# data-mermaid/mermaid-classifier

Measured on AMD Instinct MI355X. Metric: patches/sec (224x224 EfficientNet-B0), higher is better.
Workload: dtype f16; 1 GPU; EfficientNet-B0 forward, batch=256 random 224x224 u8 patches per GPU -> (256,1280) fp32; per_gpu_batch=256, global_batch=256, weights=synthetic seed 0, input_batches_rotated=8, lanes_per_gpu=2, parallelism=patch-sharded x1

## Files before the change

### include/mmc.h

```cpp
#ifndef MMC_H
#define MMC_H

#include <stddef.h>
#include <stdint.h>

#ifdef __cplusplus
extern "C" {
#endif

#define MMC_OK 0
#define MMC_ERR_ARG 1
#define MMC_ERR_WEIGHTS 2
#define MMC_ERR_HIP 3
#define MMC_ERR_NOMEM 4

#define MMC_ARCH_B0 0
#define MMC_ARCH_B4 1

#define MMC_IN_DEVICE 0u
#define MMC_IN_HOST 1u
#define MMC_OUT_DEVICE 0u
#define MMC_OUT_HOST 2u

#define MMC_FEATURE_DIM_B0 1280
#define MMC_FEATURE_DIM_B4 1792
#define MMC_PATCH 224

typedef struct mmc_backbone mmc_backbone;
typedef struct mmc_head mmc_head;

const char* mmc_last_error(void);
int mmc_version(void);
int mmc_device_count(void);

int mmc_backbone_create(const void* packed, size_t nbytes, int arch, int device, int max_batch,
                        mmc_backbone** out);
#define MMC_PRECISION_FP8 1u
int mmc_backbone_create_ex(const void* packed, size_t nbytes, int arch, int device, int max_batch, unsigned flags,
                           mmc_backbone** out);
int mmc_fp8_e4m3_encode(const float* in, uint8_t* out, size_t n);
void mmc_backbone_destroy(mmc_backbone* bb);
int mmc_feature_dim(const mmc_backbone* bb);
int mmc_backbone_max_batch(const mmc_backbone* bb);
int mmc_backbone_lanes(const mmc_backbone* bb);
size_t mmc_backbone_workspace_bytes(const mmc_backbone* bb);

int mmc_backbone_extract(mmc_backbone* bb, const void* patches, int64_t n, float* out_features,
                         unsigned flags, void* hip_stream);

int mmc_backbone_graph_stats(mmc_backbone* bb, int64_t stats[3]);

int mmc_backbone_read_activation(mmc_backbone* bb, const char* name, float* out, size_t capacity,
                                 size_t* n_written);

int mmc_backbone_profile(mmc_backbone* bb, const void* patches_dev, int64_t n, float* out_features_dev,
                         void* hip_stream, char (*names)[64], float* ms, int* launches, int cap, int* n_out);

int mmc_crop_patches(const void* image, int height, int width, const int32_t* rowcols, int64_t n,
                     void* patches_out_dev, unsigned flags, int device, void* hip_stream);

int mmc_head_create(const float* const* W, const float* const* b, const int* dims, int n_layers,
                    const float* a, const float* bcal, int K, int device, mmc_head** out);
void mmc_head_destroy(mmc_head* h);
int mmc_head_input_dim(const mmc_head* h);
int mmc_head_num_classes(const mmc_head* h);
int mmc_head_predict(mmc_head* h, const float* feats, int64_t n, float* proba, int32_t* argmax,
                     unsigned flags, void* hip_stream);

int mmc_head_topk(mmc_head* h, const float* feats, int64_t n, int k,
                  int32_t* idx , float* scores , float* proba ,
                  unsigned flags, void* hip_stream);

int mmc_classify_patches(mmc_backbone* bb, mmc_head* h, const void* patches, int64_t n, int k,
// ... 132 lines not shown
```

### mermaid_classifier_amd/_lib.py

```python

from __future__ import annotations

import ctypes as C
import os
from pathlib import Path

_HERE = Path(__file__).resolve().parent
LIB_NAME = "libmermaid_mi355.so"
LIB_PATH = _HERE / LIB_NAME

MMC_OK, MMC_ERR_ARG, MMC_ERR_WEIGHTS, MMC_ERR_HIP, MMC_ERR_NOMEM = 0, 1, 2, 3, 4
MMC_PRECISION_FP8 = 1
MMC_IN_HOST, MMC_OUT_HOST = 1, 2
MMC_EVAL_TOTALS = 5
MMC_GROUPED_MAX_BINS, MMC_COVER_SUMS = 64, 8
MMC_GROUPED_MAX_SOURCE_CELLS, MMC_GROUPED_MAX_COVER_CELLS = 1 << 26, 1 << 28
MMC_CATEGORY_MAX, MMC_CATEGORY_MAX_BINS = 64, 20
MMC_CATEGORY_MIN_BINS, MMC_CATEGORY_ROWS_PER_BIN = 2, 10
MMC_RANKED_MAX_K = 16
MMC_TRAINER_GROUP_MAX = 16

SYMBOLS = [
    "mmc_last_error", "mmc_version", "mmc_device_count",
    "mmc_backbone_create", "mmc_backbone_create_ex", "mmc_fp8_e4m3_encode", "mmc_backbone_destroy", "mmc_feature_dim", "mmc_backbone_max_batch", "mmc_backbone_lanes",
    "mmc_backbone_workspace_bytes", "mmc_backbone_extract", "mmc_backbone_read_activation",
    "mmc_backbone_profile", "mmc_backbone_graph_stats", "mmc_crop_patches",
    "mmc_head_create", "mmc_head_destroy", "mmc_head_input_dim", "mmc_head_num_classes", "mmc_head_predict", "mmc_head_topk", "mmc_classify_patches",
    "mmc_trainer_create", "mmc_trainer_destroy", "mmc_trainer_partial_fit", "mmc_trainer_partial_fit_ordered", "mmc_trainer_get_params", "mmc_trainer_adam_state",
    "mmc_trainer_logits", "mmc_trainer_evaluate", "mmc_trainer_evaluate_q32", "mmc_trainer_set_loss", "mmc_trainer_loss_gradient",
    "mmc_calibrator_create", "mmc_calibrator_destroy", "mmc_calibrator_add_features", "mmc_calibrator_add_scores", "mmc_calibrator_fit",
    "mmc_featureset_create", "mmc_featureset_destroy", "mmc_featureset_rows", "mmc_featureset_dim", "mmc_featureset_append", "mmc_featureset_read",
    "mmc_trainer_partial_fit_set", "mmc_trainer_group_partial_fit_set", "mmc_trainer_evaluate_set_q32", "mmc_calibrator_add_set",
    "mmc_trainer_evaluate_classes", "mmc_trainer_evaluate_classes_set",
    "mmc_head_evaluate", "mmc_head_evaluate_set", "mmc_head_evaluate_grouped", "mmc_head_evaluate_grouped_set",
    "mmc_head_evaluate_categories", "mmc_head_evaluate_categories_set",
    "mmc_head_evaluate_ranked", "mmc_head_evaluate_ranked_set",
    "mmc_dist_unique_id", "mmc_dist_create", "mmc_dist_destroy", "mmc_gather_features",
]


class LibraryMissingError(ImportError):
    pass


def _load() -> C.CDLL:
    path = Path(os.environ.get("MMC_LIBRARY", LIB_PATH))
    if not path.is_file():
        raise LibraryMissingError(
            f"{path} not found: build it with `python -m mermaid_classifier_amd.build` "
            "(hipcc --offload-arch=gfx950). mermaid_classifier_amd has no CPU fallback.")
    try:
        import torch
    except ImportError:
        pass
    lib = C.CDLL(str(path))
    vp, i32, i64, u32, sz = C.c_void_p, C.c_int, C.c_int64, C.c_uint, C.c_size_t
    fp = C.POINTER(C.c_float)
    lib.mmc_last_error.restype = C.c_char_p
    lib.mmc_last_error.argtypes = []
    lib.mmc_version.restype = i32
    lib.mmc_device_count.restype = i32
    lib.mmc_backbone_create.restype = i32
    lib.mmc_backbone_create.argtypes = [vp, sz, i32, i32, i32, C.POINTER(vp)]
    lib.mmc_backbone_create_ex.restype = i32
    lib.mmc_backbone_create_ex.argtypes = [vp, sz, i32, i32, i32, u32, C.POINTER(vp)]
    lib.mmc_fp8_e4m3_encode.restype = i32
    lib.mmc_fp8_e4m3_encode.argtypes = [vp, vp, sz]
    lib.mmc_backbone_destroy.restype = None
    lib.mmc_backbone_destroy.argtypes = [vp]
    lib.mmc_feature_dim.restype = i32
    lib.mmc_feature_dim.argtypes = [vp]
    lib.mmc_backbone_max_batch.restype = i32
    lib.mmc_backbone_max_batch.argtypes = [vp]
    lib.mmc_backbone_lanes.restype = i32
    lib.mmc_backbone_lanes.argtypes = [vp]
    lib.mmc_backbone_workspace_bytes.restype = sz
    lib.mmc_backbone_workspace_bytes.argtypes = [vp]
    lib.mmc_backbone_extract.restype = i32
    lib.mmc_backbone_extract.argtypes = [vp, vp, i64, vp, u32, vp]
    lib.mmc_backbone_read_activation.restype = i32
    lib.mmc_backbone_read_activation.argtypes = [vp, C.c_char_p, vp, sz, C.POINTER(sz)]
    lib.mmc_backbone_profile.restype = i32
    lib.mmc_backbone_profile.argtypes = [vp, vp, i64, vp, vp, vp, fp, C.POINTER(i32), i32, C.POINTER(i32)]
    lib.mmc_backbone_graph_stats.restype = i32
    lib.mmc_backbone_graph_stats.argtypes = [vp, C.POINTER(i64)]
    lib.mmc_crop_patches.restype = i32
    lib.mmc_crop_patches.argtypes = [vp, i32, i32, vp, i64, vp, u32, i32, vp]
    lib.mmc_head_create.restype = i32
    lib.mmc_head_create.argtypes = [C.POINTER(fp), C.POINTER(fp), C.POINTER(i32), i32, fp, fp, i32, i32, C.POINTER(vp)]
    lib.mmc_head_destroy.restype = None
    lib.mmc_head_destroy.argtypes = [vp]
    lib.mmc_head_input_dim.restype = i32
    lib.mmc_head_input_dim.argtypes = [vp]
    lib.mmc_head_num_classes.restype = i32
    lib.mmc_head_num_classes.argtypes = [vp]
    lib.mmc_head_predict.restype = i32
    lib.mmc_head_predict.argtypes = [vp, vp, i64, vp, vp, u32, vp]
    lib.mmc_head_topk.restype = i32
    lib.mmc_head_topk.argtypes = [vp, vp, i64, i32, vp, vp, vp, u32, vp]
    lib.mmc_classify_patches.restype = i32
# ... 110 lines not shown
```

### mermaid_classifier_amd/csrc/device_common.h

```cpp
#pragma once
#include <hip/hip_runtime.h>
#include <stdint.h>
#include <stdlib.h>
#include <algorithm>
#include <atomic>
#include <type_traits>

#include "kernels.h"

typedef _Float16 h8 __attribute__((ext_vector_type(8)));
typedef _Float16 h4 __attribute__((ext_vector_type(4)));
typedef float f4 __attribute__((ext_vector_type(4)));
typedef float f2 __attribute__((ext_vector_type(2)));

static __device__ __forceinline__ float sigmoid_f(float x) { return __builtin_amdgcn_rcpf(1.0f + __expf(-x)); }
static __device__ __forceinline__ float silu_f(float x) { return x * sigmoid_f(x); }
static __device__ __forceinline__ float silu_scaled(float t)
{
    return t * __builtin_amdgcn_rcpf(1.0f + __builtin_amdgcn_exp2f(-t));
}

static __device__ __forceinline__ uint32_t cvt_pk_f16(float a, float b)
{
    uint32_t d;
// ... 69 lines not shown
}

static __device__ __forceinline__ float fma_mix_lo(uint32_t h2, float w, float acc)
{
    float d;
    asm("v_fma_mix_f32 %0, %1, %2, %3 op_sel_hi:[1,0,0]" : "=v"(d) : "v"(h2), "v"(w), "v"(acc));
    return d;
}
static __device__ __forceinline__ float fma_mix_hi(uint32_t h2, float w, float acc)
{
    float d;
    asm("v_fma_mix_f32 %0, %1, %2, %3 op_sel:[1,0,0] op_sel_hi:[1,0,0]" : "=v"(d) : "v"(h2), "v"(w), "v"(acc));
    return d;
}


#define GLOBAL_AS __attribute__((address_space(1)))
typedef uint32_t u2v __attribute__((ext_vector_type(2)));
typedef uint32_t u4v __attribute__((ext_vector_type(4)));
template <typename T>
static __device__ __forceinline__ const GLOBAL_AS T* sgpr_ptr(const void* p)
{
    const uint64_t v = reinterpret_cast<uint64_t>(p);
    const uint32_t lo = __builtin_amdgcn_readfirstlane((uint32_t)v), hi = __builtin_amdgcn_readfirstlane((uint32_t)(v >> 32));
    return reinterpret_cast<const GLOBAL_AS T*>(((uint64_t)hi << 32) | lo);
}
template <typename T>
static __device__ __forceinline__ T gload(const GLOBAL_AS void* base, unsigned byte_off)
{
    return *reinterpret_cast<const GLOBAL_AS T*>(reinterpret_cast<const GLOBAL_AS char*>(base) + byte_off);
}
#define T7_BAR() asm volatile("s_waitcnt lgkmcnt(0)\n\ts_barrier" ::: "memory")

#define LAUNCH_CHECK()                          \
    do {                                        \
        hipError_t e__ = hipGetLastError();     \
        if (e__ != hipSuccess) return (int)e__; \
    } while (0)

template <auto Kernel>
static int set_max_lds(int bytes)
{
    static std::atomic<bool> done[64];
    int dev = 0;
    if (hipGetDevice(&dev) != hipSuccess) dev = 0;
    const bool tracked = dev >= 0 && dev < 64;
    if (tracked && done[dev].load(std::memory_order_acquire)) return 0;
    const hipError_t e = hipFuncSetAttribute(reinterpret_cast<const void*>(Kernel), hipFuncAttributeMaxDynamicSharedMemorySize, bytes);
    if (e != hipSuccess) return (int)e;
    if (tracked) done[dev].store(true, std::memory_order_release);
    return 0;
}

template <int NK, typename Args>
struct Inst {
    int key[NK];
    const char* label;
    int (*launch)(const Args&, hipStream_t);
};
template <int NK, typename Args, size_t N>
static const Inst<NK, Args>* find_inst(const Inst<NK, Args> (&table)[N], const int (&key)[NK])
{
    for (const auto& t : table)
        if (std::equal(key, key + NK, t.key)) return &t;
    return nullptr;
}
// ... 14 lines not shown
```

### mermaid_classifier_amd/csrc/k_early.hip

```cpp
#include "device_common.h"

template <int KSTEPS, bool RES>
__global__ __launch_bounds__(256) void thin_proj_kernel(const _Float16* __restrict__ X, int K, const _Float16* __restrict__ Wp,
                                                        const float* __restrict__ bias, _Float16* __restrict__ Y, int N,
                                                        const float* __restrict__ gate, int HW, int frags_per_wg,
                                                        const _Float16* __restrict__ res, int plane_rows)
{
    const int tid = threadIdx.x, lane = tid & 63, wave = tid >> 6;
    const int m = lane & 15, q = lane >> 4;
    const int b = blockIdx.y;
    const int nfrag = HW >> 4;
    const int f0 = blockIdx.x * frags_per_wg;
    const int f1 = f0 + frags_per_wg < nfrag ? f0 + frags_per_wg : nfrag;
    const int cbase = q * 8;
    const int cres = cbase < N ? cbase : 0;
    const _Float16* xb = X + (size_t)b * HW * K;
    auto load = [&](int f, h8 (&dst)[KSTEPS], h8& r) {
        const size_t row = (size_t)f * 16 + m;
#pragma unroll
        for (int ks = 0; ks < KSTEPS; ++ks) {
            const int k0 = ks * 32 + q * 8, k = k0 < K ? k0 : K - 8;
            dst[ks] = plane_rows ? *reinterpret_cast<const h8*>(X + (((size_t)(k >> 5) * plane_rows + (size_t)b * HW + row) * 32 + (k & 31)))
                                 : *reinterpret_cast<const h8*>(xb + row * K + k);
        }
// ... 30 lines not shown
        if (more) load(f + 4, xn, rn);
        f4 a0 = bv0, a1 = bv1;
#pragma unroll
        for (int ks = 0; ks < KSTEPS; ++ks) {
            a0 = __builtin_amdgcn_mfma_f32_16x16x32_f16(wf[ks][0], xc[ks], a0, 0, 0, 0);
            a1 = __builtin_amdgcn_mfma_f32_16x16x32_f16(wf[ks][1], xc[ks], a1, 0, 0, 0);
        }
        if (cbase < N) {
            h8 o;
#pragma unroll
            for (int j = 0; j < 4; ++j) {
                o[j] = (_Float16)(a0[j] + (RES ? (float)rc[j] : 0.f));
                o[4 + j] = (_Float16)(a1[j] + (RES ? (float)rc[4 + j] : 0.f));
            }
            *reinterpret_cast<h8*>(Y + ((size_t)b * HW + (size_t)f * 16 + m) * N + cbase) = o;
        }
        if (more) {
#pragma unroll
            for (int ks = 0; ks < KSTEPS; ++ks) xc[ks] = xn[ks];
            rc = rn;
        }
    }
}

template <bool PLANAR>
__global__ __launch_bounds__(512, 4) void mb1_kernel(Mb1Args a)
{
    constexpr int WC = 58, NPOS = 17 * WC, NPF = (NPOS + 15) / 16, ES2 = 160;
    extern __shared__ __attribute__((aligned(16))) unsigned char smem[];
    unsigned char* E = smem;
    float* pred = reinterpret_cast<float*>(smem + NPF * 8 * ES2);
    const int tid = threadIdx.x, lane = tid & 63, wave = __builtin_amdgcn_readfirstlane(tid >> 6);
    const int m = lane & 15, q = lane >> 4;
    const int tile = blockIdx.x, b = blockIdx.z;
    const int ty = tile >> 1, tx = tile & 1;
    const int oy0 = 8 * ty, ox0 = 28 * tx, iy0 = 16 * ty, ix0 = 56 * tx;
    const GLOBAL_AS _Float16* xg = sgpr_ptr<_Float16>(a.X) + (size_t)b * 112 * 112 * 32;
    uint2 xbp[8];
    {
        u4v xr[8];
#pragma unroll
        for (int i = 0; i < 8; ++i) {
            const int pf = wave + 8 * i;
            const int p = 16 * pf + m;
            const int r = p / WC, c = p - r * WC;
            const int iy = iy0 + r, ix = ix0 + c;
            const bool ok = pf < NPF && p < NPOS && iy < 112 && ix < 112;
            xr[i] = gload<u4v>(xg, (unsigned)((((ok ? iy : 0) * 112 + (ok ? ix : 0)) * 32 + 8 * q) * 2));
        }
        const uint4 wraw = *reinterpret_cast<const uint4*>(a.pre_w + lane * 8);
        const f4 bpre = *reinterpret_cast<const f4*>(a.pre_b + 4 * q);
        const f4 g0 = *reinterpret_cast<const f4*>(a.pre_gate + (size_t)b * 32 + 8 * q);
        const f4 g1 = *reinterpret_cast<const f4*>(a.pre_gate + (size_t)b * 32 + 8 * q + 4);
        const uint4 wgated = gate_h8(wraw, g0, g1);
        const h8 wpre = *reinterpret_cast<const h8*>(&wgated);
#pragma unroll
        for (int i = 0; i < 8; ++i) {
            const f4 x1 = __builtin_amdgcn_mfma_f32_16x16x32_f16(wpre, *reinterpret_cast<const h8*>(&xr[i]), bpre, 0, 0, 0);
            h4 xh;
#pragma unroll
            for (int j = 0; j < 4; ++j) xh[j] = (_Float16)x1[j];
            xbp[i] = *reinterpret_cast<const uint2*>(&xh);
        }
    }
    h4 wexp[2];
    float bexp[2];
    float kdw[9], dbias;
// ... 85 lines not shown
            for (int j = 0; j < 14; j += 2) {
                const f2 v = {acc[j], acc[j + 1]};
                psum2 = psum2 + v;
                const uint32_t hv = cvt_pk_f16(acc[j], acc[j + 1]);
                dg[(size_t)j * PS] = (uint16_t)hv;
                dg[(size_t)(j + 1) * PS] = (uint16_t)(hv >> 16);
            }
            pred[(tid >> 5) * 32 + c] = psum2.x + psum2.y;
        }
        T7_BAR();
        if (tid < 32) {
            float s = 0.f;
#pragma unroll
            for (int w = 0; w < 16; ++w) s += pred[w * 32 + tid];
            a.pool[((size_t)b * 14 + tile) * 96 + chunk * 32 + tid] = s;
        }
    }
}

template <int KSD, int CKS, int CE, int HIMG>
__global__ __launch_bounds__(512) void mbt_kernel(MbtArgs a)
{
    constexpr int R = KSD / 2, NP = KSD == 5 ? 3 : 2, NROWS = 14 + 2 * R, CH = 48;
    constexpr int ES2 = 224;
    constexpr int WW = HIMG == 28 ? 28 : 30;
    constexpr int NPOS = NROWS * WW, NPF = (NPOS + 15) / 16;
    static_assert(NPF <= 32, "four fragments per wave");
    constexpr int TX = HIMG / 28, NR = 3 + 2 * R;
    extern __shared__ __attribute__((aligned(16))) unsigned char smem[];
    unsigned char* E = smem;
    float* pred = reinterpret_cast<float*>(smem + NPF * 8 * ES2);
    const int tid = threadIdx.x, lane = tid & 63, wave = __builtin_amdgcn_readfirstlane(tid >> 6);
    const int m = lane & 15, q = lane >> 4;
    const int tile = blockIdx.x, chunk = blockIdx.y, b = blockIdx.z;
    const int ty = tile / TX, tx = tile - ty * TX;
    const int oy0 = 14 * ty, ox0 = 28 * tx;
    const int wx0 = ox0 >= 2 ? ox0 - 2 : 0;
    const int Cin = a.Cin;
    const GLOBAL_AS _Float16* xg = sgpr_ptr<_Float16>(a.X) + (size_t)b * HIMG * HIMG * Cin;
    const GLOBAL_AS _Float16* wexp = sgpr_ptr<_Float16>(a.wexp);
    uint32_t raw[15];
    float dbias;
    const int cg_dw = chunk * CH + tid % CH;
    {
        u4v xr[4][CKS];
        constexpr bool MASK_E = KSD != 3;
        bool okp[4][2];
#pragma unroll
        for (int i = 0; i < 4; ++i) {
            const int p = 16 * (wave + 8 * i) + m;
            const int r = p / WW, c = p - r * WW;
            const int iy = oy0 - R + r, ix = wx0 + c;
            const bool ok = p < NPOS && iy >= 0 && iy < HIMG && ix < HIMG;
            const int row = ok ? iy * HIMG + ix : 0;
#pragma unroll
            for (int h = 0; h < 2; ++h) {
                const int pp = 16 * (wave + 8 * i) + 4 * q + 2 * h;
                const int pr = pp / WW, pc = pp - pr * WW;
                const int py = oy0 - R + pr;
                okp[i][h] = !MASK_E || (pp < NPOS && py >= 0 && py < HIMG && wx0 + pc < HIMG);
            }
#pragma unroll
            for (int ks = 0; ks < CKS; ++ks) {
                const int kk = 32 * ks + 8 * q;
                xr[i][ks] = gload<u4v>(xg, (unsigned)((row * Cin + (kk < Cin ? kk : Cin - 8)) * 2));
            }
        }
// ... 86 lines not shown
                            const bool out = ro == 0 ? (oy0 + rb == 0) : (oy0 + rb + 1 == HIMG - 1);
                            wq[0][0] = out ? 0u : wq[0][0]; wq[0][1] = out ? 0u : wq[0][1];
                            wq[1][0] = out ? 0u : wq[1][0]; wq[1][1] = out ? 0u : wq[1][1];
                        }
                    }
#pragma unroll
                    for (int ip = 0; ip < NP; ++ip)
#pragma unroll
                        for (int j = 0; j < 14; ++j) {
                            const int l = (KSD == 5 || !(j & 1)) ? (j >> 1) + ip : (j >> 1) + 1 + ip;
                            if (ky == 0 && ip == 0) acc[j] = dot2_from(P[ro + ky][l], wq[j & 1][ip], dbias);
                            else acc[j] = __builtin_amdgcn_fdot2(*reinterpret_cast<const h2*>(&P[ro + ky][l]),
                                                                 *reinterpret_cast<const h2*>(&wq[j & 1][ip]), acc[j], false);
                        }
                }
                silu_scaled_staged(acc);
#pragma unroll
                for (int j = 0; j < 14; j += 2) {
                    const f2 v = {acc[j], acc[j + 1]};
                    psum2 = psum2 + v;
                    const uint32_t hv = cvt_pk_f16(acc[j], acc[j + 1]);
                    reinterpret_cast<uint16_t*>(dg)[((size_t)ro * HIMG + j) * CE] = (uint16_t)hv;
                    reinterpret_cast<uint16_t*>(dg)[((size_t)ro * HIMG + j + 1) * CE] = (uint16_t)(hv >> 16);
                }
            }
        }
        pred[rest * CH + c] = psum2.x + psum2.y;
    }
    T7_BAR();
    if (tid < CH) {
        float s = 0.f;
#pragma unroll
        for (int w = 0; w < 10; ++w) s += pred[w * CH + tid];
        a.pool[((size_t)b * gridDim.x + tile) * CE + chunk * CH + tid] = s;
    }
}

template <int CKS, int CE>
__global__ __launch_bounds__(512, 4) void mbt4_kernel(MbtArgs a)
{
    constexpr int HIMG = 28, R = 2, KSD = 5, NROWS = 18, WW = 28, CH = 48, NPOS = NROWS * WW, NPF = 32;
    constexpr int ERS = 64, ECS = 1160;
    constexpr int TREG = 56 * 32;
    extern __shared__ __attribute__((aligned(16))) unsigned char smem[];
    unsigned char* E = smem;
    const int tid = threadIdx.x, lane = tid & 63, wave = __builtin_amdgcn_readfirstlane(tid >> 6);
    unsigned char* TW = smem + CH * ECS + wave * TREG;
    float* pred = reinterpret_cast<float*>(smem + CH * ECS + 8 * TREG);
    const int m = lane & 15, q = lane >> 4;
    const int tile = blockIdx.x, chunk = blockIdx.y, b = blockIdx.z;
    const int oy0 = 14 * tile;
    const int Cin = a.Cin;
    const GLOBAL_AS _Float16* xg = sgpr_ptr<_Float16>(a.X) + (size_t)b * HIMG * HIMG * Cin;
    const GLOBAL_AS _Float16* wexp = sgpr_ptr<_Float16>(a.wexp);
    const GLOBAL_AS _Float16* dwt = sgpr_ptr<_Float16>(a.dwtoe);
    {
        u4v xr[4][CKS];
        int eoff[4];
        bool okq[4];
#pragma unroll
        for (int i = 0; i < 4; ++i) {
            const int p = 16 * (wave + 8 * i) + m;
            const int r = (p * 2341) >> 16, c = p - r * WW;
            const int iy = oy0 - R + r;
            const bool ok = p < NPOS && iy >= 0 && iy < HIMG;
            const int row = ok ? iy * HIMG + c : 0;
            const int pq = 16 * (wave + 8 * i) + 4 * q;
            const int qr = (pq * 2341) >> 16, qc = pq - qr * WW;
            const int qy = oy0 - R + qr;
            okq[i] = pq < NPOS && qy >= 0 && qy < HIMG;
            eoff[i] = pq < NPOS ? qr * ERS + qc * 2 : NROWS * ERS;
#pragma unroll
            for (int ks = 0; ks < CKS; ++ks) {
                const int kk = 32 * ks + 8 * q;
                xr[i][ks] = gload<u4v>(xg, (unsigned)((row * Cin + (kk < Cin ? kk : Cin - 8)) * 2));
            }
        }
        h8 wa[3][CKS];
        float ba[3];
#pragma unroll
        for (int nf = 0; nf < 3; ++nf) {
            const int nfg = 3 * chunk + nf;
#pragma unroll
// ... 98 lines not shown
            }
            float v[14];
#pragma unroll
            for (int x = 0; x < 14; ++x) v[x] = XH == 0 ? acc[(x + 2) >> 2][(x + 2) & 3] : acc[x >> 2][x & 3];
            silu_scaled_staged(v);
            float s = ((v[0] + v[1]) + (v[2] + v[3])) + ((v[4] + v[5]) + (v[6] + v[7])) + ((v[8] + v[9]) + (v[10] + v[11])) + (v[12] + v[13]);
            s = quad_sum(rowok ? s : 0.f);
            if (n == 0) pred[(2 * yt + xh) * CH + 16 * g + c] = s;
#pragma unroll
            for (int j = 0; j < 7; ++j) {
                float lo = v[j], hi = v[7 + j];
                asm volatile("s_nop 1\n\tv_permlane16_swap_b32 %0, %1\n\ts_nop 1" : "+v"(lo), "+v"(hi));
                *reinterpret_cast<uint32_t*>(tst + j * 32) = cvt_pk_f16(lo, hi);
            }
#pragma unroll
            for (int rr = 0; rr < 2; ++rr) {
                const uint4 o = *reinterpret_cast<const uint4*>(TW + toff[rr]);
                *reinterpret_cast<uint4*>(dgb + goff[rr] + 32 * g) = o;
            }
        };
        if (xh == 0) {
#pragma unroll
            for (int g = 0; g < 3; ++g) item(g, std::integral_constant<int, 0>{});
        } else {
#pragma unroll
            for (int g = 0; g < 3; ++g) item(g, std::integral_constant<int, 1>{});
        }
    }
    T7_BAR();
    if (tid < CH) {
        float s = 0.f;
#pragma unroll
        for (int w = 0; w < 8; ++w) s += pred[w * CH + tid];
        a.pool[((size_t)b * gridDim.x + tile) * CE + chunk * CH + tid] = s;
    }
}

template <int KSD, int CKS, int CE, int HIMG>
__global__ __launch_bounds__(512) void mbt2_kernel(MbtArgs a)
{
    constexpr int PADB = KSD == 5 ? 1 : 0, NIP = KSD == 5 ? 3 : 2, NROWS = 12 + KSD, CH = 48, ES2 = 224;
    constexpr int WW = KSD == 5 ? 32 : 30, NPOS = NROWS * WW, NPF = (NPOS + 15) / 16, NS = (NPF + 7) / 8;
    constexpr int HOUT = HIMG / 2, TX = HOUT / 14, NPR = KSD == 5 ? 16 : 15;
    extern __shared__ __attribute__((aligned(16))) unsigned char smem[];
    unsigned char* E = smem;
    float* pred = reinterpret_cast<float*>(smem + NS * 64 * ES2);
    const int tid = threadIdx.x, lane = tid & 63, wave = __builtin_amdgcn_readfirstlane(tid >> 6);
    const int m = lane & 15, q = lane >> 4;
    const int tile = blockIdx.x, chunk = blockIdx.y, b = blockIdx.z;
    const int ty = tile / TX, tx = tile - ty * TX;
    const int oy0 = 7 * ty, ox0 = 14 * tx;
    const int wy0 = 2 * oy0 - PADB;
    int wx0 = (2 * ox0 - PADB) & ~1;
    wx0 = wx0 < 0 ? 0 : wx0;
    const int pbase = (2 * ox0 - PADB - wx0 - (KSD == 5 ? 1 : 0)) >> 1;
    const int Cin = a.Cin;
    const GLOBAL_AS _Float16* xg = sgpr_ptr<_Float16>(a.X) + (size_t)b * HIMG * HIMG * Cin;
    const GLOBAL_AS _Float16* wexp = sgpr_ptr<_Float16>(a.wexp);
    uint32_t raw[15];
    float dbias;
    const int cg_dw = chunk * CH + tid % CH;
    {
        u4v xr[NS][CKS];
        constexpr bool MASK_E = KSD != 3;
        static_assert(KSD != 3 || HIMG == 28, "the 3x3 stride-2 shortcut assumes one tile column");
        bool okp[NS][2];
#pragma unroll
        for (int i = 0; i < NS; ++i) {
            const int p = 16 * (wave + 8 * i) + m;
            const int r = p / WW, c = p - r * WW;
            const int iy = wy0 + r, ix = wx0 + c;
            const bool ok = p < NPOS && iy >= 0 && iy < HIMG && ix < HIMG;
            const int row = ok ? iy * HIMG + ix : 0;
#pragma unroll
            for (int h = 0; h < 2; ++h) {
                const int pp = 16 * (wave + 8 * i) + 4 * q + 2 * h;
                const int pr = pp / WW, pc = pp - pr * WW;
                const int py = wy0 + pr;
                okp[i][h] = !MASK_E || (pp < NPOS && py >= 0 && py < HIMG && wx0 + pc < HIMG);
            }
#pragma unroll
            for (int ks = 0; ks < CKS; ++ks) {
// ... 82 lines not shown
                    const bool out = oy0 + orow == HOUT - 1;
                    wq[0] = out ? 0u : wq[0]; wq[1] = out ? 0u : wq[1];
                }
                wql = half ? 0u : wq[1];
            }
#pragma unroll
            for (int ip = 0; ip < NIP; ++ip)
#pragma unroll
                for (int j = 0; j < 7; ++j) {
                    const uint32_t wt = (KSD == 3 && j == 6 && ip == 1) ? wql : wq[ip];
                    if (ky == 0 && ip == 0) acc[j] = dot2_from(P[ky][j + ip], wt, dbias);
                    else acc[j] = __builtin_amdgcn_fdot2(*reinterpret_cast<const h2*>(&P[ky][j + ip]), *reinterpret_cast<const h2*>(&wt), acc[j], false);
                }
        }
        f2 psum2 = {0.f, 0.f};
        uint16_t* dg = reinterpret_cast<uint16_t*>(a.D + (((size_t)b * HOUT + oy0 + orow) * HOUT + ox0 + 7 * half) * CE + cg);
        silu_scaled_staged(acc);
#pragma unroll
        for (int j = 0; j < 6; j += 2) {
            const f2 v = {acc[j], acc[j + 1]};
            psum2 = psum2 + v;
            const uint32_t hv = cvt_pk_f16(acc[j], acc[j + 1]);
            dg[(size_t)j * CE] = (uint16_t)hv;
            dg[(size_t)(j + 1) * CE] = (uint16_t)(hv >> 16);
        }
        reinterpret_cast<_Float16*>(dg)[(size_t)6 * CE] = (_Float16)acc[6];
        pred[rest * CH + c] = (psum2.x + psum2.y) + acc[6];
    }
    T7_BAR();
    if (tid < CH) {
        float s = 0.f;
#pragma unroll
        for (int w = 0; w < 14; ++w) s += pred[w * CH + tid];
        a.pool[((size_t)b * gridDim.x + tile) * CE + chunk * CH + tid] = s;
    }
}

#define SD_T 16
#define SD_WIN (SD_T + 2)
#define SD_IN (2 * SD_WIN + 1)
#define SD_ROWH 128
#define SD_ES 80
__global__ __launch_bounds__(256) void stem_dw_kernel(const uint8_t* __restrict__ patches,
                                                      const _Float16* __restrict__ w,
                                                      const float* __restrict__ bias,
                                                      const float* __restrict__ padval,
                                                      const float* __restrict__ Wdw,
                                                      const float* __restrict__ bdw,
                                                      _Float16* __restrict__ out,
                                                      float* __restrict__ pool_part)
{
    __shared__ __attribute__((aligned(16))) _Float16 tile[SD_IN * SD_ROWH];
    __shared__ __attribute__((aligned(16))) unsigned char E[((SD_WIN * SD_WIN + 15) / 16 * 16) * SD_ES];
    __shared__ __attribute__((aligned(16))) float wl[9 * 32];
    const int tx = blockIdx.x, ty = blockIdx.y, b = blockIdx.z;
    const int tid = threadIdx.x, lane = tid & 63, wave = tid >> 6;
    const int m = lane & 15, q = lane >> 4;
    const int oy0 = ty * SD_T, ox0 = tx * SD_T;
    int wy0 = oy0 - 1, wy1 = oy0 + SD_T + 1, wx0 = ox0 - 1, wx1 = ox0 + SD_T + 1;
    wy0 = wy0 < 0 ? 0 : wy0;
    wx0 = wx0 < 0 ? 0 : wx0;
    wy1 = wy1 > 112 ? 112 : wy1;
    wx1 = wx1 > 112 ? 112 : wx1;
    const int wh = wy1 - wy0;
    constexpr int P = SD_WIN * SD_WIN;
    const int dy = wy0 - (oy0 - 1);
    const int icol0 = 2 * (ox0 - 2);
    constexpr int cshift = 2;
    h8 wf[2];
#pragma unroll
    for (int t = 0; t < 2; ++t) wf[t] = *reinterpret_cast<const h8*>(w + (t * 16 + m) * 32 + q * 8);
    f4 bsv[2];
#pragma unroll
    for (int t = 0; t < 2; ++t) bsv[t] = *reinterpret_cast<const f4*>(bias + q * 8 + t * 4);
    const f4 bdw0 = *reinterpret_cast<const f4*>(bdw + (tid & 3) * 8), bdw1 = *reinterpret_cast<const f4*>(bdw + (tid & 3) * 8 + 4);
    const float wl0 = Wdw[tid], wl1 = Wdw[256 + (tid & 31)];
    {
        const uint8_t* img = patches + (size_t)b * (224 * 224 * 3);
        const int iy0 = 2 * wy0;
        const int rows = 2 * wh + 1;
        const float pv0 = padval[0], pv1 = padval[1], pv2 = padval[2];
        const bool interior = tx < 6 && ty < 6;
        if (interior) {
            constexpr int NIT = (37 * 31 + 255) / 256;
            uint32_t wd[NIT];
            const int nd = rows * 31;
#pragma unroll
            for (int it = 0; it < NIT; ++it) {
// ... 169 lines not shown
        pool_part[((size_t)b * 49 + ty * 7 + tx) * 32 + tid] = sum;
    }
}

template <int KSTEPS, bool RES>
static int launch_thin_proj_t(const GemmArgs& a, hipStream_t st)
{
    const int nfrag = a.HW / 16, patches = a.M / a.HW;
    int per = (int)(((long)nfrag * patches / 2048 + 3) / 4 * 4);
    if (per < 8) per = 8;
    if (per > 112) per = 112;
    if (nfrag < per) per = nfrag;
    dim3 grid((nfrag + per - 1) / per, patches);
    hipLaunchKernelGGL((thin_proj_kernel<KSTEPS, RES>), grid, dim3(256), 0, st, a.X, a.K, a.Wp, a.bias, a.Y, a.N, a.gate, a.HW, per, a.res,
                       a.x_plane_rows);
    LAUNCH_CHECK();
    return 0;
}

#define TP(KSTEPS, RES) {{KSTEPS, RES}, "thin_proj", launch_thin_proj_t<KSTEPS, RES != 0>},
static const Inst<2, GemmArgs> THIN_PROJ_TABLE[] = {TP(1, 1) TP(2, 0) TP(3, 0) TP(5, 0) TP(5, 1)};
#undef TP

const char* thin_proj_label(int ksteps, int res) { return inst_label(THIN_PROJ_TABLE, {ksteps, res}); }

int launch_thin_proj(const GemmArgs& a, int patches, hipStream_t st)
{
    if (a.nt != 2 || a.n_chunks != 1 || a.K > 192 || (a.K & 7) || a.N > 32 || (a.N & 7) || (a.HW & 15) || !a.gate || a.epi != EPI_LINEAR ||
        a.M != patches * a.HW || (a.x_plane_rows && (a.x_plane_rows != a.M || (a.K & 31))))
        return -15;
    return inst_launch(THIN_PROJ_TABLE, {a.Kp / 32, a.res ? 1 : 0}, a, st, -15);
}

int launch_stem_dw(const uint8_t* patches, const _Float16* w, const float* bias, const float* padval, const float* Wdw,
                   const float* bdw, _Float16* out, float* pool_part, int B, hipStream_t st)
{
    hipLaunchKernelGGL(stem_dw_kernel, dim3(7, 7, B), dim3(256), 0, st, patches, w, bias, padval, Wdw, bdw, out, pool_part);
    LAUNCH_CHECK();
    return 0;
}

int launch_mb1(const Mb1Args& a, hipStream_t st)
{
    if (a.B < 1) return -15;
    const int lds = 62 * 8 * 160 + 16 * 32 * 4;
    if (int r = set_max_lds<&mb1_kernel<false>>(lds)) return r;
    if (int r = set_max_lds<&mb1_kernel<true>>(lds)) return r;
    if (a.planar) hipLaunchKernelGGL(mb1_kernel<true>, dim3(14, 1, a.B), dim3(512), lds, st, a);
    else hipLaunchKernelGGL(mb1_kernel<false>, dim3(14, 1, a.B), dim3(512), lds, st, a);
    LAUNCH_CHECK();
    return 0;
}

template <int KSD, int CKS, int CE, int HIMG>
static int launch_mbt_t(const MbtArgs& a, hipStream_t st)
{
    constexpr int NROWS = 14 + 2 * (KSD / 2), WW = HIMG == 28 ? 28 : 30, NPF = (NROWS * WW + 15) / 16;
    const int lds = NPF * 16 * 112 + 10 * 48 * 4;
    if (int r = set_max_lds<&mbt_kernel<KSD, CKS, CE, HIMG>>(lds)) return r;
    hipLaunchKernelGGL((mbt_kernel<KSD, CKS, CE, HIMG>), dim3((HIMG / 14) * (HIMG / 28), CE / 48, a.B), dim3(512), lds, st, a);
    LAUNCH_CHECK();
    return 0;
}

template <int CKS, int CE>
static int launch_mbt4_t(const MbtArgs& a, hipStream_t st)
{
    const int lds = 48 * 1160 + 8 * 56 * 32 + 8 * 48 * 4;
    if (int r = set_max_lds<&mbt4_kernel<CKS, CE>>(lds)) return r;
    hipLaunchKernelGGL((mbt4_kernel<CKS, CE>), dim3(2, CE / 48, a.B), dim3(512), lds, st, a);
    LAUNCH_CHECK();
    return 0;
}

template <int KSD, int CKS, int CE, int HIMG>
static int launch_mbt2_t(const MbtArgs& a, hipStream_t st)
{
    constexpr int NROWS = 12 + KSD, WW = KSD == 5 ? 32 : 30, NPF = (NROWS * WW + 15) / 16, NS = (NPF + 7) / 8, HOUT = HIMG / 2;
    const int lds = NS * 64 * 224 + 14 * 48 * 4;
    if (int r = set_max_lds<&mbt2_kernel<KSD, CKS, CE, HIMG>>(lds)) return r;
    hipLaunchKernelGGL((mbt2_kernel<KSD, CKS, CE, HIMG>), dim3((HOUT / 7) * (HOUT / 14), CE / 48, a.B), dim3(512), lds, st, a);
    LAUNCH_CHECK();
    return 0;
}

#define MBT(KSD, CKS, CE, HIMG, CIN) {{HIMG, KSD, 1, CIN, CE, 0}, "mbt<" #KSD "," #CKS "," #CE "," #HIMG ">", launch_mbt_t<KSD, CKS, CE, HIMG>},
#define MBT2(KSD, CKS, CE, HIMG, CIN) {{HIMG, KSD, 2, CIN, CE, 0}, "mbt2<" #KSD "," #CKS "," #CE "," #HIMG ">", launch_mbt2_t<KSD, CKS, CE, HIMG>},
#define MBT4(CKS, CE, CIN) {{28, 5, 1, CIN, CE, 1}, "mbt4<" #CKS "," #CE ">", launch_mbt4_t<CKS, CE>},
static const Inst<6, MbtArgs> MBT_TABLE[] = {
    MBT(3, 1, 144, 56, 24)
    MBT(5, 2, 240, 28, 40)
    MBT4(2, 240, 40)
    MBT2(5, 1, 144, 56, 24)
    MBT2(3, 2, 240, 28, 40)
    MBT(3, 1, 192, 56, 32)
    MBT(5, 2, 336, 28, 56)
    MBT4(2, 336, 56)
    MBT2(5, 1, 192, 56, 32)
    MBT2(3, 2, 336, 28, 56)
};
#undef MBT4
#undef MBT2
#undef MBT

const char* mbt_label(int H, int ks, int stride, int Cin, int Ce, int dw4) { return inst_label(MBT_TABLE, {H, ks, stride, Cin, Ce, dw4}); }

int launch_mbt(const MbtArgs& a, hipStream_t st)
{
    if (a.B < 1) return -16;
    return inst_launch(MBT_TABLE, {a.H, a.ks, a.stride, a.Cin, a.Ce, a.dwtoe ? 1 : 0}, a, st, -5);
}
```

### mermaid_classifier_amd/csrc/kernels.h

```cpp
#pragma once
#include <hip/hip_runtime.h>
#include <stdint.h>

enum { EPI_SILU = 0, EPI_LINEAR = 1, EPI_GAP = 2 };


int mmc_fail(int code, const char* fmt, ...);

struct GemmArgs {
    const _Float16* X;
    int M, K;
    const _Float16* Wp;
    int Kp;
    const float* bias;
    _Float16* Y;
    int N;
    int mt, nt, n_chunks, defer_gate;
    int epi;
    const float* gate;
    int HW;
    const _Float16* res;
    float* gap_out;
    int x_plane_rows;
    float inv_hw;
// ... 149 lines not shown
    float psc;
};
int launch_proj_patch(const ProjPatchArgs& a, hipStream_t st);
int proj_patch_ksteps(int K);
int proj_patch_fc1_rows(int K);
const char* proj_patch_label(int K, int N, int HW, int res);

enum { CHAIN14_MAX_PHASES = 7 };
struct Chain14Phase {
    int kind;
    union {
        ProjPatchArgs pp;
        Mid14Args mid;
    };
};
struct Chain14Args {
    int B, nph;
    Chain14Phase ph[CHAIN14_MAX_PHASES];
};
int chain14_proj_kind(int K, int N, int HW, int res);
int chain14_mid_kind(int Cin, int ks, int Ce);
int launch_chain14(const Chain14Args& a, hipStream_t st);

int launch_mbconv_a(const MbArgs& a, hipStream_t st);
const char* mbconv_a_label(const MbArgs& a);
const char* mbconv_pre_label(const MbArgs& a);
const char* mbconv_d_label(const MbArgs& a);
int launch_mbconv_pre(const MbArgs& a, const _Float16* pre_w, const float* pre_b, const float* pre_gate, hipStream_t st);
int launch_mbconv_d(const MbArgs& a, hipStream_t st);
int launch_stem(const uint8_t* patches, const _Float16* w, const float* bias, const float* padval, _Float16* out, int B,
                int channels, hipStream_t st);
int launch_stem_dw(const uint8_t* patches, const _Float16* w, const float* bias, const float* padval, const float* Wdw,
                   const float* bdw, _Float16* out, float* pool_part, int B, hipStream_t st);
int launch_pw_gemm(const GemmArgs& a, hipStream_t st);
const char* pw_gemm_label(int mt, int nt, int epi, int gate, int res, int defer_gate);
int launch_thin_proj(const GemmArgs& a, int patches, hipStream_t st);
const char* thin_proj_label(int ksteps, int res);
int launch_dwconv(const DwArgs& a, hipStream_t st);
const char* dwconv_label(int ks, int stride, int tw);
int launch_se_gate(const float* pool_part, int nparts, int B, int C, int Cs4, const float* WrP, const float* br,
                   const float* WeP, const float* be, float* gate, hipStream_t st);
int launch_se_small(const float* pool_part, int nparts, int B, int C, int Cs, const float* wr, const float* br,
                    const float* we, const float* be, float* gate, hipStream_t st);
int launch_se_wide(const float* pool_part, int nparts, int B, int C, int Cs, const float* wr, const float* br,
                   const float* we_t , const float* be, float* gate, hipStream_t st);
int launch_mlp_layer(const float* X, int M, int K, const float* W, const float* bias, float* Y, int N, bool relu,
                     hipStream_t st);
int launch_calibrate(const float* logits, int M, int K, const float* a, const float* b, float* proba, int32_t* argmax,
                     hipStream_t st);
int launch_calibrate_topk(const float* logits, int M, int K, const float* a, const float* b, int k, int32_t* idx, float* scores,
                          float* proba, float* rowbuf, hipStream_t st);
constexpr int EVAL_TOTALS = 5;
int launch_calibrate_eval(const float* logits, int M, int K, const float* a, const float* b, const int32_t* y, const int32_t* label_map,
                          int n_labels, int32_t* est, float* score, int32_t* rank, float* p_true, long long* totals, long long* confusion,
                          long long* rank_hist, int32_t* scored, float* rowbuf, hipStream_t st);
constexpr int RANK_MAX_K = 16;
int launch_rank_rows(const float* logits, int M, int K, const float* a, const float* b, const int32_t* scored, const int32_t* rank,
                     const uint8_t* sim_level, int n_levels, int kmax, long long* class_rank_hist, long long* hier_hist, float* rowbuf,
                     hipStream_t st);
int launch_crop(const uint8_t* image, int H, int W, const int32_t* rowcols, int n, uint8_t* out, hipStream_t st);

constexpr int GROUP_MAX_BINS = 64;
constexpr int GROUP_MAX_TARGETS = 2 * GROUP_MAX_BINS;
constexpr int GROUP_HIST_WORDS = GROUP_MAX_TARGETS * 1024;
constexpr uint32_t GROUP_KEY_NONE = 0xFFFFFFFFu;
constexpr int GROUP_MAX_CATEGORIES = 64;
// ... 31 lines not shown
```

### mermaid_classifier_amd/csrc/mmc_api.cpp

```cpp
#include <hip/hip_runtime.h>

#include <algorithm>
#include <cmath>
#include <cstdarg>
#include <cstdio>
#include <cstdlib>
#include <cstring>
#include <map>
#include <mutex>
#include <thread>
#include <string>
#include <vector>

#include "../../include/mmc.h"
#include "api_internal.h"
#include "kernels.h"

static thread_local char g_err[512] = "";

int mmc_fail(int code, const char* fmt, ...)
{
    va_list ap;
    va_start(ap, fmt);
    vsnprintf(g_err, sizeof g_err, fmt, ap);
// ... 59 lines not shown
struct PwLayer {
    int N = 0, K = 0, Kp = 0, nt = 0, n_chunks = 0;
    _Float16* w = nullptr;
    float* b = nullptr;
    const char* label[2] = {nullptr, nullptr};
};

struct Fp8Layer {
    int N = 0, K = 0, KS128 = 0, NFp = 0;
    uint8_t* w8 = nullptr;
    float* sw = nullptr;
    float* b = nullptr;
};

static uint8_t e4m3_encode(float x)
{
    if (x != x) return 0x7F;
    const uint8_t sign = std::signbit(x) ? 0x80 : 0x00;
    float a = std::fabs(x);
    if (a >= 448.0f) return sign | 0x7E;
    if (a < 0.0009765625f) return sign;
    int e;
    (void)std::frexp(a, &e);
    int ex = e - 1;
    if (ex < -6) ex = -6;
    const float quantum = std::ldexp(1.0f, ex - 3);
    float qf = std::nearbyint(a / quantum);
    int qi = (int)qf;
    if (qi >= 16) { qi = 8; ++ex; }
    if (ex > 8) return sign | 0x7E;
    if (ex == 8 && qi > 14) return sign | 0x7E;
    if (qi < 8) return sign | (uint8_t)qi;
    return sign | (uint8_t)(((ex + 7) << 3) | (qi - 8));
}

extern "C" int mmc_fp8_e4m3_encode(const float* in, uint8_t* out, size_t n)
{
    if (!in || !out) return fail(MMC_ERR_ARG, "NULL argument");
    for (size_t i = 0; i < n; ++i) out[i] = e4m3_encode(in[i]);
    return MMC_OK;
}

static int pick_nt(int N, bool small_m)
{
    const int tiles = (N + 15) / 16;
    if (small_m) {
        int best = 4, waste = 1 << 30;
        for (int nt = 4; nt >= 2; --nt) {
            const int w = (tiles + nt - 1) / nt * nt - tiles;
            if (w < waste) { waste = w; best = nt; }
        }
        return tiles <= 4 ? tiles : best;
    }
    for (int nt = 8; nt >= 1; --nt)
        if (tiles % nt == 0) return nt;
    return 1;
}

struct Options {
    bool keep, graph, tail_clk, profile_serial;
    bool fuse, fuse_b0, mb1, mbt, mbt2, mbt4, mb_dot2, mid14, mid14m, projse, se_small, thin_proj, b1_planar;
    bool tail, tail_full, tail_b11;
    bool chain;
    int lanes, fp8_maxh;
};
static bool env_starts(const char* name, char c)
// ... 1483 lines not shown
```

Before: 243,000 patches/s.

## Remap early-stage workgroups so consecutive IDs interleave eight patches

Early-stage kernels (stem_dw, mb1, mbt, mbt4, mbt2) switch from a 3D grid (tile, chunk, batch) to a 1D grid. Each group of eight consecutive workgroup IDs now covers the same tile/chunk across eight different patches. The goal is to spread concurrently dispatched workgroups across patches and XCDs, and to let workgroups that share weights for the same tile/chunk run together, improving cache locality and load balance. It also adds a host-side helper and API export that reports the mapping, plus bounds checks for padded patches, at the cost of a few idle workgroups when B is not a multiple of eight.

```diff
diff --git a/include/mmc.h b/include/mmc.h
--- a/include/mmc.h
+++ b/include/mmc.h
@@ -39,6 +39,7 @@
 int mmc_backbone_create_ex(const void* packed, size_t nbytes, int arch, int device, int max_batch, unsigned flags,
                            mmc_backbone** out);
 int mmc_fp8_e4m3_encode(const float* in, uint8_t* out, size_t n);
+int mmc_patch_affine_map(int n_patches, int wgs_per_patch, int* patch, int* index, int cap, int* grid);
 void mmc_backbone_destroy(mmc_backbone* bb);
 int mmc_feature_dim(const mmc_backbone* bb);
 int mmc_backbone_max_batch(const mmc_backbone* bb);
diff --git a/mermaid_classifier_amd/_lib.py b/mermaid_classifier_amd/_lib.py
--- a/mermaid_classifier_amd/_lib.py
+++ b/mermaid_classifier_amd/_lib.py
@@ -22,7 +22,7 @@
 
 SYMBOLS = [
     "mmc_last_error", "mmc_version", "mmc_device_count",
-    "mmc_backbone_create", "mmc_backbone_create_ex", "mmc_fp8_e4m3_encode", "mmc_backbone_destroy", "mmc_feature_dim", "mmc_backbone_max_batch", "mmc_backbone_lanes",
+    "mmc_backbone_create", "mmc_backbone_create_ex", "mmc_fp8_e4m3_encode", "mmc_patch_affine_map", "mmc_backbone_destroy", "mmc_feature_dim", "mmc_backbone_max_batch", "mmc_backbone_lanes",
     "mmc_backbone_workspace_bytes", "mmc_backbone_extract", "mmc_backbone_read_activation",
     "mmc_backbone_profile", "mmc_backbone_graph_stats", "mmc_crop_patches",
     "mmc_head_create", "mmc_head_destroy", "mmc_head_input_dim", "mmc_head_num_classes", "mmc_head_predict", "mmc_head_topk", "mmc_classify_patches",
@@ -66,6 +66,8 @@
     lib.mmc_backbone_create_ex.argtypes = [vp, sz, i32, i32, i32, u32, C.POINTER(vp)]
     lib.mmc_fp8_e4m3_encode.restype = i32
     lib.mmc_fp8_e4m3_encode.argtypes = [vp, vp, sz]
+    lib.mmc_patch_affine_map.restype = i32
+    lib.mmc_patch_affine_map.argtypes = [i32, i32, vp, vp, i32, C.POINTER(i32)]
     lib.mmc_backbone_destroy.restype = None
     lib.mmc_backbone_destroy.argtypes = [vp]
     lib.mmc_feature_dim.restype = i32
diff --git a/mermaid_classifier_amd/csrc/device_common.h b/mermaid_classifier_amd/csrc/device_common.h
--- a/mermaid_classifier_amd/csrc/device_common.h
+++ b/mermaid_classifier_amd/csrc/device_common.h
@@ -125,6 +125,16 @@
 }
 #define T7_BAR() asm volatile("s_waitcnt lgkmcnt(0)\n\ts_barrier" ::: "memory")
 
+struct PatchWg {
+    int b, w;
+};
+static __host__ __device__ __forceinline__ PatchWg patch_affine(int id, int W)
+{
+    const int r = id >> 3, g = r / W;
+    return {8 * g + (id & 7), r - g * W};
+}
+static inline int patch_affine_grid(int B, int W) { return 8 * W * ((B + 7) / 8); }
+
 #define LAUNCH_CHECK()                          \
     do {                                        \
         hipError_t e__ = hipGetLastError();     \
diff --git a/mermaid_classifier_amd/csrc/k_early.hip b/mermaid_classifier_amd/csrc/k_early.hip
--- a/mermaid_classifier_amd/csrc/k_early.hip
+++ b/mermaid_classifier_amd/csrc/k_early.hip
@@ -86,7 +86,9 @@
     float* pred = reinterpret_cast<float*>(smem + NPF * 8 * ES2);
     const int tid = threadIdx.x, lane = tid & 63, wave = __builtin_amdgcn_readfirstlane(tid >> 6);
     const int m = lane & 15, q = lane >> 4;
-    const int tile = blockIdx.x, b = blockIdx.z;
+    const PatchWg pw = patch_affine(blockIdx.x, 14);
+    if (pw.b >= a.B) return;
+    const int tile = pw.w, b = pw.b;
     const int ty = tile >> 1, tx = tile & 1;
     const int oy0 = 8 * ty, ox0 = 28 * tx, iy0 = 16 * ty, ix0 = 56 * tx;
     const GLOBAL_AS _Float16* xg = sgpr_ptr<_Float16>(a.X) + (size_t)b * 112 * 112 * 32;
@@ -238,7 +240,10 @@
     float* pred = reinterpret_cast<float*>(smem + NPF * 8 * ES2);
     const int tid = threadIdx.x, lane = tid & 63, wave = __builtin_amdgcn_readfirstlane(tid >> 6);
     const int m = lane & 15, q = lane >> 4;
-    const int tile = blockIdx.x, chunk = blockIdx.y, b = blockIdx.z;
+    constexpr int NT = (HIMG / 14) * TX, NC = CE / CH;
+    const PatchWg pw = patch_affine(blockIdx.x, NT * NC);
+    if (pw.b >= a.B) return;
+    const int tile = pw.w / NC, chunk = pw.w - tile * NC, b = pw.b;
     const int ty = tile / TX, tx = tile - ty * TX;
     const int oy0 = 14 * ty, ox0 = 28 * tx;
     const int wx0 = ox0 >= 2 ? ox0 - 2 : 0;
@@ -391,7 +396,7 @@
         float s = 0.f;
 #pragma unroll
         for (int w = 0; w < 10; ++w) s += pred[w * CH + tid];
-        a.pool[((size_t)b * gridDim.x + tile) * CE + chunk * CH + tid] = s;
+        a.pool[((size_t)b * NT + tile) * CE + chunk * CH + tid] = s;
     }
 }
 
@@ -407,7 +412,10 @@
     unsigned char* TW = smem + CH * ECS + wave * TREG;
     float* pred = reinterpret_cast<float*>(smem + CH * ECS + 8 * TREG);
     const int m = lane & 15, q = lane >> 4;
-    const int tile = blockIdx.x, chunk = blockIdx.y, b = blockIdx.z;
+    constexpr int NT = 2, NC = CE / CH;
+    const PatchWg pw = patch_affine(blockIdx.x, NT * NC);
+    if (pw.b >= a.B) return;
+    const int tile = pw.w / NC, chunk = pw.w - tile * NC, b = pw.b;
     const int oy0 = 14 * tile;
     const int Cin = a.Cin;
     const GLOBAL_AS _Float16* xg = sgpr_ptr<_Float16>(a.X) + (size_t)b * HIMG * HIMG * Cin;
@@ -572,7 +580,7 @@
         float s = 0.f;
 #pragma unroll
         for (int w = 0; w < 8; ++w) s += pred[w * CH + tid];
-        a.pool[((size_t)b * gridDim.x + tile) * CE + chunk * CH + tid] = s;
+        a.pool[((size_t)b * NT + tile) * CE + chunk * CH + tid] = s;
     }
 }
 
@@ -587,7 +595,10 @@
     float* pred = reinterpret_cast<float*>(smem + NS * 64 * ES2);
     const int tid = threadIdx.x, lane = tid & 63, wave = __builtin_amdgcn_readfirstlane(tid >> 6);
     const int m = lane & 15, q = lane >> 4;
-    const int tile = blockIdx.x, chunk = blockIdx.y, b = blockIdx.z;
+    constexpr int NT = (HOUT / 7) * TX, NC = CE / CH;
+    const PatchWg pw = patch_affine(blockIdx.x, NT * NC);
+    if (pw.b >= a.B) return;
+    const int tile = pw.w / NC, chunk = pw.w - tile * NC, b = pw.b;
     const int ty = tile / TX, tx = tile - ty * TX;
     const int oy0 = 7 * ty, ox0 = 14 * tx;
     const int wy0 = 2 * oy0 - PADB;
@@ -736,7 +747,7 @@
         float s = 0.f;
 #pragma unroll
         for (int w = 0; w < 14; ++w) s += pred[w * CH + tid];
-        a.pool[((size_t)b * gridDim.x + tile) * CE + chunk * CH + tid] = s;
+        a.pool[((size_t)b * NT + tile) * CE + chunk * CH + tid] = s;
     }
 }
 
@@ -752,12 +763,15 @@
                                                       const float* __restrict__ Wdw,
                                                       const float* __restrict__ bdw,
                                                       _Float16* __restrict__ out,
-                                                      float* __restrict__ pool_part)
+                                                      float* __restrict__ pool_part,
+                                                      int B)
 {
     __shared__ __attribute__((aligned(16))) _Float16 tile[SD_IN * SD_ROWH];
     __shared__ __attribute__((aligned(16))) unsigned char E[((SD_WIN * SD_WIN + 15) / 16 * 16) * SD_ES];
     __shared__ __attribute__((aligned(16))) float wl[9 * 32];
-    const int tx = blockIdx.x, ty = blockIdx.y, b = blockIdx.z;
+    const PatchWg pw = patch_affine(blockIdx.x, 49);
+    if (pw.b >= B) return;
+    const int ty = pw.w / 7, tx = pw.w - 7 * ty, b = pw.b;
     const int tid = threadIdx.x, lane = tid & 63, wave = tid >> 6;
     const int m = lane & 15, q = lane >> 4;
     const int oy0 = ty * SD_T, ox0 = tx * SD_T;
@@ -993,10 +1007,22 @@
     return inst_launch(THIN_PROJ_TABLE, {a.Kp / 32, a.res ? 1 : 0}, a, st, -15);
 }
 
+int patch_affine_map(int B, int W, int* patch, int* index, int cap)
+{
+    const int n = patch_affine_grid(B, W);
+    for (int id = 0; id < n && id < cap; ++id) {
+        const PatchWg pw = patch_affine(id, W);
+        patch[id] = pw.b;
+        index[id] = pw.w;
+    }
+    return n;
+}
+
 int launch_stem_dw(const uint8_t* patches, const _Float16* w, const float* bias, const float* padval, const float* Wdw,
                    const float* bdw, _Float16* out, float* pool_part, int B, hipStream_t st)
 {
-    hipLaunchKernelGGL(stem_dw_kernel, dim3(7, 7, B), dim3(256), 0, st, patches, w, bias, padval, Wdw, bdw, out, pool_part);
+    if (B < 1) return -15;
+    hipLaunchKernelGGL(stem_dw_kernel, dim3(patch_affine_grid(B, 49)), dim3(256), 0, st, patches, w, bias, padval, Wdw, bdw, out, pool_part, B);
     LAUNCH_CHECK();
     return 0;
 }
@@ -1007,8 +1033,9 @@
     const int lds = 62 * 8 * 160 + 16 * 32 * 4;
     if (int r = set_max_lds<&mb1_kernel<false>>(lds)) return r;
     if (int r = set_max_lds<&mb1_kernel<true>>(lds)) return r;
-    if (a.planar) hipLaunchKernelGGL(mb1_kernel<true>, dim3(14, 1, a.B), dim3(512), lds, st, a);
-    else hipLaunchKernelGGL(mb1_kernel<false>, dim3(14, 1, a.B), dim3(512), lds, st, a);
+    const dim3 grid(patch_affine_grid(a.B, 14));
+    if (a.planar) hipLaunchKernelGGL(mb1_kernel<true>, grid, dim3(512), lds, st, a);
+    else hipLaunchKernelGGL(mb1_kernel<false>, grid, dim3(512), lds, st, a);
     LAUNCH_CHECK();
     return 0;
 }
@@ -1019,7 +1046,7 @@
     constexpr int NROWS = 14 + 2 * (KSD / 2), WW = HIMG == 28 ? 28 : 30, NPF = (NROWS * WW + 15) / 16;
     const int lds = NPF * 16 * 112 + 10 * 48 * 4;
     if (int r = set_max_lds<&mbt_kernel<KSD, CKS, CE, HIMG>>(lds)) return r;
-    hipLaunchKernelGGL((mbt_kernel<KSD, CKS, CE, HIMG>), dim3((HIMG / 14) * (HIMG / 28), CE / 48, a.B), dim3(512), lds, st, a);
+    hipLaunchKernelGGL((mbt_kernel<KSD, CKS, CE, HIMG>), dim3(patch_affine_grid(a.B, (HIMG / 14) * (HIMG / 28) * (CE / 48))), dim3(512), lds, st, a);
     LAUNCH_CHECK();
     return 0;
 }
@@ -1029,7 +1056,7 @@
 {
     const int lds = 48 * 1160 + 8 * 56 * 32 + 8 * 48 * 4;
     if (int r = set_max_lds<&mbt4_kernel<CKS, CE>>(lds)) return r;
-    hipLaunchKernelGGL((mbt4_kernel<CKS, CE>), dim3(2, CE / 48, a.B), dim3(512), lds, st, a);
+    hipLaunchKernelGGL((mbt4_kernel<CKS, CE>), dim3(patch_affine_grid(a.B, 2 * (CE / 48))), dim3(512), lds, st, a);
     LAUNCH_CHECK();
     return 0;
 }
@@ -1040,7 +1067,7 @@
     constexpr int NROWS = 12 + KSD, WW = KSD == 5 ? 32 : 30, NPF = (NROWS * WW + 15) / 16, NS = (NPF + 7) / 8, HOUT = HIMG / 2;
     const int lds = NS * 64 * 224 + 14 * 48 * 4;
     if (int r = set_max_lds<&mbt2_kernel<KSD, CKS, CE, HIMG>>(lds)) return r;
-    hipLaunchKernelGGL((mbt2_kernel<KSD, CKS, CE, HIMG>), dim3((HOUT / 7) * (HOUT / 14), CE / 48, a.B), dim3(512), lds, st, a);
+    hipLaunchKernelGGL((mbt2_kernel<KSD, CKS, CE, HIMG>), dim3(patch_affine_grid(a.B, (HOUT / 7) * (HOUT / 14) * (CE / 48))), dim3(512), lds, st, a);
     LAUNCH_CHECK();
     return 0;
 }
diff --git a/mermaid_classifier_amd/csrc/kernels.h b/mermaid_classifier_amd/csrc/kernels.h
--- a/mermaid_classifier_amd/csrc/kernels.h
+++ b/mermaid_classifier_amd/csrc/kernels.h
@@ -205,6 +205,7 @@
                 int channels, hipStream_t st);
 int launch_stem_dw(const uint8_t* patches, const _Float16* w, const float* bias, const float* padval, const float* Wdw,
                    const float* bdw, _Float16* out, float* pool_part, int B, hipStream_t st);
+int patch_affine_map(int B, int W, int* patch, int* index, int cap);
 int launch_pw_gemm(const GemmArgs& a, hipStream_t st);
 const char* pw_gemm_label(int mt, int nt, int epi, int gate, int res, int defer_gate);
 int launch_thin_proj(const GemmArgs& a, int patches, hipStream_t st);
diff --git a/mermaid_classifier_amd/csrc/mmc_api.cpp b/mermaid_classifier_amd/csrc/mmc_api.cpp
--- a/mermaid_classifier_amd/csrc/mmc_api.cpp
+++ b/mermaid_classifier_amd/csrc/mmc_api.cpp
@@ -115,6 +115,15 @@
     if (ex == 8 && qi > 14) return sign | 0x7E;
     if (qi < 8) return sign | (uint8_t)qi;
     return sign | (uint8_t)(((ex + 7) << 3) | (qi - 8));
+}
+
+extern "C" int mmc_patch_affine_map(int n_patches, int wgs_per_patch, int* patch, int* index, int cap, int* grid)
+{
+    if (!patch || !index || !grid) return fail(MMC_ERR_ARG, "NULL argument");
+    if (n_patches < 1 || wgs_per_patch < 1 || cap < 0 || (int64_t)wgs_per_patch * (n_patches + 7) > INT32_MAX)
+        return fail(MMC_ERR_ARG, "mmc_patch_affine_map: %d patches x %d workgroups out of range", n_patches, wgs_per_patch);
+    *grid = patch_affine_map(n_patches, wgs_per_patch, patch, index, cap);
+    return MMC_OK;
 }
 
 extern "C" int mmc_fp8_e4m3_encode(const float* in, uint8_t* out, size_t n)
```

Measured after the change: 243,300 patches/s (median of 6 runs). Within noise of the previous version (+0.1%).
